# andr345/frtm-vos

Measured on AMD Instinct MI355X. Metric: segmented frames/sec/GPU (480p, ResNet101, full CG iters), higher is better.
Workload: dtype f32

## Files before the change

### frtm-vos_amd/_hip.py

```python
import ctypes
import os

import torch

_HERE = os.path.dirname(os.path.abspath(__file__))
LIB_PATH = os.path.join(_HERE, 'libfrtm_hip.so')

P, I, F, D = ctypes.c_void_p, ctypes.c_int, ctypes.c_float, ctypes.c_double


class ConvDesc(ctypes.Structure):
    _fields_ = [(k, I) for k in ('B', 'Cin', 'Hin', 'Win', 'Cout', 'ksize', 'stride', 'pad',
                                 'relu', 'out_transposed', 'splitk', 'tile', 'w_layout', 'ws_elems', 'w_pitch')]


SIGNATURES = {
    'frtm_last_error': (ctypes.c_char_p, []),
    'frtm_version': (I, []),
    'frtm_device_info': (I, [P]),
    'frtm_pixel_weights': (I, [P, I, I, I, I, F, P, P, P]),
    'frtm_normal_build': (I, [P, I, P, I, I, I, I, I, F, P, I, P, P, P, P, P]),
    'frtm_memory_next_slot': (I, [P, I, F, I, P, P, I, P]),
    'frtm_memory_insert': (I, [P, P, I, P, P]),
    'frtm_filter_scores': (I, [P, P, I, I, I, I, P, I, P]),
# ... 82 lines not shown
    'frtm_bn_stats': (I, [P, I, I, I, F, F, I, P, P, P, P, P, P]),
    'frtm_bn_apply_relu': (I, [P, P, P, P, P, I, I, I, P, P]),
    'frtm_bn_relu_backward': (I, [P, P, P, P, P, P, I, I, I, I, P, P, P, P, P]),
    'frtm_relu_backward': (I, [P, P, ctypes.c_size_t, P, P]),
    'frtm_pyrup2x_backward': (I, [P, I, I, I, P, P, P]),
    'frtm_bilinear_backward': (I, [P, I, I, I, I, I, P, P, P]),
    'frtm_cab_backward_reduce': (I, [P, P, I, I, P, P, P]),
    'frtm_cab_gate_backward': (I, [P, P, P, P, P, P, P, P, I, I, P, P, P, P, P, P, P]),
    'frtm_cab_backward_shallow': (I, [P, P, P, I, I, P, P]),
    'frtm_add_plane': (I, [P, P, F, I, I, P]),
    'frtm_shift9': (I, [P, I, I, I, P, P]),
    'frtm_cab_gate': (I, [P, P, I, P, P, P, P, I, I, P, P]),
    'frtm_project_tail_fits': (I, [I, I, I, I, I]),
    'frtm_project_tail': (I, [P, I, I, I, I, P, P, I, I, P, P]),
    'frtm_tap_mix': (I, [P, I, I, I, P, P, P]),
    'frtm_bicubic_resize': (I, [P, I, I, I, P, I, I, P]),
    'frtm_project_tail_bicubic': (I, [P, I, I, I, I, P, P, I, I, P, P]),
    'frtm_warp_affine': (I, [P, I, I, I, P, I, I, P, I, P]),
    'frtm_warp_affine_u8': (I, [P, I, I, I, P, I, I, P, I, P]),
    'frtm_warp_mask_batch': (I, [P, I, I, P, I, I, P, I, P, P]),
    'frtm_fill32': (I, [P, ctypes.c_size_t, ctypes.c_uint, P]),
    'frtm_label_mask': (I, [P, I, ctypes.c_size_t, P, P, P]),
    'frtm_mask_stats': (I, [P, I, I, I, P, P]),
    'frtm_aug_prepare': (I, [P, P, I, I, P, P, P, P, P]),
    'frtm_pull_push_fill': (I, [P, ctypes.c_size_t, I, I, P]),
    'frtm_pull_push_elems': (ctypes.c_size_t, [I, I]),
    'frtm_aug_transforms': (I, [P, I, P, I, I, P, P, P]),
    'frtm_warp_mask_batch_dev': (I, [P, I, I, P, I, I, P, I, P, P]),
    'frtm_warp_affine_batch': (I, [P, I, I, I, P, I, I, P, P, I, P]),
    'frtm_aug_blend': (I, [P, P, I, I, I, P, P, P, P, P]),
# ... 247 lines not shown
```

### frtm-vos_amd/build.py

```python
import os
import subprocess
import sys

HERE = os.path.dirname(os.path.abspath(__file__))
CSRC = os.path.join(HERE, 'csrc')
LIB = os.path.join(HERE, 'libfrtm_hip.so')
SOURCES = ['target_model.hip', 'target_apply_grouped.hip', 'cg_persistent.hip', 'joint_persistent.hip', 'joint_fit.hip', 'wide_maps.hip', 'conv_igemm.hip', 'conv_gemm32.hip', 'conv_wino.hip', 'conv_wino4.hip', 'conv_bf16x3.hip', 'conv_bf16x1.hip', 'conv3x3_bf16x1.hip', 'conv3x3s2_bf16x1.hip', 'conv_wgrad_bf16x1.hip', 'backbone.hip', 'image_ops.hip', 'refiner_ops.hip', 'refiner_train.hip', 'ragged_group.hip', 'telea_host.hip', 'jf_eval.hip', 'train_step.hip', 'frame_resize.hip', 'native_size.hip']
HIPCC = os.environ.get('HIPCC', '/opt/rocm/bin/hipcc')
FLAGS = ['--offload-arch=gfx950', '-O3', '-std=c++17', '-fPIC', '-Wall', '-Wno-unused-function']
if os.environ.get('FRTM_BUILD_ABLATE'):
    FLAGS.append('-DFRTM_DEBUG_ABLATE')


def _stale(target, deps):
    if not os.path.exists(target):
        return True
    t = os.path.getmtime(target)
    return any(os.path.getmtime(d) > t for d in deps)


def build(force=False, verbose=True):
    headers = [os.path.join(CSRC, 'frtm_common.h'), os.path.join(CSRC, 'conv_common.h'), os.path.join(CSRC, 'resident_grid.h'), os.path.join(CSRC, 'resample_taps.h'), os.path.join(CSRC, 'trunk_route.h'), os.path.join(os.path.dirname(HERE), 'include', 'frtm_hip.h'), __file__]
    objs = []
    for src in SOURCES:
        sp = os.path.join(CSRC, src)
        if not os.path.exists(sp):
            continue
        obj = os.path.join(CSRC, src.replace('.hip', '.o'))
        objs.append(obj)
        if force or _stale(obj, [sp] + headers):
            cmd = [HIPCC] + FLAGS + ['-c', sp, '-o', obj]
            if verbose:
                print(' '.join(cmd), flush=True)
            subprocess.check_call(cmd)
    if force or _stale(LIB, objs):
        cmd = [HIPCC, '--offload-arch=gfx950', '-shared', '-fPIC'] + objs + ['-o', LIB]
        if verbose:
# ... 8 lines not shown
```

### frtm-vos_amd/csrc/refiner_ops.hip

```cpp
#include "frtm_common.h"
#include "resample_taps.h"
#include "../../include/frtm_hip.h"

__global__ __launch_bounds__(256) void k_bilinear_resize(const float* __restrict__ in, int h, int w, float* __restrict__ out, int H, int W,
                                                          int planes, int planes_per_z) {
  const int pix = blockIdx.x * 256 + threadIdx.x;
  if (pix >= H * W) return;
  const int y = pix / W, x = pix - y * W;
  int y0, y1, x0, x1; float ly0, ly1, lx0, lx1;
  bilinear_taps(y, (float)h / (float)H, h, y0, y1, ly0, ly1);
  bilinear_taps(x, (float)w / (float)W, w, x0, x1, lx0, lx1);
  const float w00 = ly0 * lx0, w01 = ly0 * lx1, w10 = ly1 * lx0, w11 = ly1 * lx1;
  const int o00 = y0 * w + x0, o01 = y0 * w + x1, o10 = y1 * w + x0, o11 = y1 * w + x1;
  const int p0 = blockIdx.y * planes_per_z, p1 = min(planes, p0 + planes_per_z);
  const size_t hw = (size_t)h * w, HW = (size_t)H * W;
  for (int pl = p0; pl < p1; ++pl) {
    const float* p = in + pl * hw;
    out[pl * HW + pix] = w00 * p[o00] + w01 * p[o01] + w10 * p[o10] + w11 * p[o11];
  }
}

#define INJ_TH 8
#define INJ_TW 32
#define INJ_CG 4
// ... 143 lines not shown
  const float* p = in + (size_t)blockIdx.x * HW;
  float acc = 0.f;
  if ((HW & 3) == 0 && ((size_t)p & 15) == 0) {
    const float4* p4 = (const float4*)p;
    float a0 = 0.f, a1 = 0.f, a2 = 0.f, a3 = 0.f;
    for (int i = threadIdx.x; i < HW / 4; i += 256) { const float4 v = p4[i]; a0 += v.x; a1 += v.y; a2 += v.z; a3 += v.w; }
    acc = (a0 + a1) + (a2 + a3);
  } else {
    for (int i = threadIdx.x; i < HW; i += 256) acc += p[i];
  }
  acc = block_sum(acc, red);
  if (threadIdx.x == 0) out[blockIdx.x] = acc / (float)HW;
}


#define PT_TH 16
#define PT_TW 64
#define PT_UR 22
#define PT_UC 76
#define PT_YR (PT_UR / 2 + 5)
#define PT_YC (PT_UC / 2 + 5)
#define PT_ZR (PT_TH + 2)
#define PT_ZC (PT_TW + 2)
#define PT_CG 2

__device__ __forceinline__ float pyr_taps(int odd, float a, float b, float c, float d) {
  const float E0 = PYR2X_E0, E1 = PYR2X_E1, E2 = PYR2X_E2, E3 = PYR2X_E3;
  return odd ? E0 * a + E1 * b + E2 * c + E3 * d : E3 * a + E2 * b + E1 * c + E0 * d;
}

__global__ __launch_bounds__(256, 4) void k_project_tail(const float* __restrict__ y, int C, int h, int w, const float* __restrict__ wgt,
                                                       const float* __restrict__ bias, float* __restrict__ out, int Ho, int Wo) {
  constexpr int NY = PT_YR * PT_YC, NYL = (PT_CG * NY + 255) / 256;
  constexpr int NZ = PT_ZR * PT_ZC, NZL = (NZ + 255) / 256;
  __shared__ float ybuf[PT_CG][PT_YR][PT_YC];
  __shared__ float ub[PT_CG][PT_UR][PT_UC];
  __shared__ float zb[PT_CG][PT_ZR][PT_ZC + 1];
  __shared__ int ri0[PT_ZR], ri1[PT_ZR], cj0[PT_ZC], cj1[PT_ZC];
  __shared__ float rl0[PT_ZR], rl1[PT_ZR], cl0[PT_ZC], cl1[PT_ZC];
  __shared__ int org[2];
  const int tid = threadIdx.x, n = blockIdx.z;
  const int Y0 = blockIdx.y * PT_TH, X0 = blockIdx.x * PT_TW;
  const int Hu = 2 * h, Wu = 2 * w;
  if (tid < PT_ZR) {
// ... 413 lines not shown
```

### frtm-vos_amd/csrc/target_model.hip

```cpp
#include "frtm_common.h"
#include "resample_taps.h"
#include "../../include/frtm_hip.h"

__device__ __forceinline__ void hinge_weights(float px, float HW, float tf, float& wf, float& wb) {
  if (tf < 0.f) { wf = 1.f; wb = 1.f; return; }
  float af = px / HW;
  if (px < 10.f) af = tf;
  const float tfe = (af > tf) ? af : tf;
  wf = tfe / af;
  wb = (1.f - tfe) / (1.f - af);
}

template <bool U8>
__device__ __forceinline__ float load_label(const void* p, size_t i) {
  if (U8) return (float)((const unsigned char*)p)[i];
  return ((const float*)p)[i];
}

template <bool U8, bool THRESH>
__global__ __launch_bounds__(256) void k_label_sum(const void* __restrict__ y, int HW, float* __restrict__ partial) {
  __shared__ float red[16];
  const int n = blockIdx.y, part = blockIdx.x;
  const size_t base = (size_t)n * HW;
  const int per = (HW + FRTM_PX_PARTS - 1) / FRTM_PX_PARTS;
// ... 652 lines not shown
__global__ __launch_bounds__(256) void k_transpose2d(const float* __restrict__ in, int rows, int cols, float* __restrict__ out) {
  __shared__ float tile[32][33];
  const int bx = blockIdx.x * 32, by = blockIdx.y * 32;
  const int tx = threadIdx.x & 31, ty = threadIdx.x >> 5;
  for (int k = ty; k < 32; k += 8) {
    const int r = by + k, c = bx + tx;
    tile[k][tx] = (r < rows && c < cols) ? in[(size_t)r * cols + c] : 0.f;
  }
  __syncthreads();
  for (int k = ty; k < 32; k += 8) {
    const int c = bx + k, r = by + tx;
    if (r < rows && c < cols) out[(size_t)c * rows + r] = tile[tx][k];
  }
}

#define MERGE_MAX 16
__global__ __launch_bounds__(256) void k_merge_masks(float* __restrict__ masks, int K, int HW) {
  masks += (size_t)blockIdx.y * K * HW;
  for (int i = blockIdx.x * 256 + threadIdx.x; i < HW; i += gridDim.x * 256) {
    float p[MERGE_MAX];
    float bg = INFINITY;
    for (int k = 1; k < K; ++k) {
      float v = masks[(size_t)k * HW + i];
      v = fminf(fmaxf(v, 1e-7f), 1.f - 1e-7f);
      p[k] = v;
      bg = fminf(bg, 1.f - v);
    }
    p[0] = bg;
    float mx = -INFINITY; int arg = 0;
    for (int k = 0; k < K; ++k) { p[k] = p[k] / (1.f - p[k]); if (p[k] > mx) { mx = p[k]; arg = k; } }
    float den = 0.f;
// ... 46 lines not shown
  if (threadIdx.x == 0) {
    const int tot = (wsum[0] + wsum[1]) + (wsum[2] + wsum[3]);
    if (tot) atomicAdd(&count[k], tot);
  }
}

__global__ __launch_bounds__(256) void k_track_merge(const float* __restrict__ logits, int n, int HW, float* __restrict__ masks,
                                                     unsigned char* __restrict__ labels, const unsigned char* __restrict__ lut, int single,
                                                     int* __restrict__ counts, float thr) {
  const int K = n + 1, f = blockIdx.y;
  logits += (size_t)f * n * HW;
  masks += (size_t)f * K * HW;
  int cnt[MERGE_MAX];
#pragma unroll
  for (int k = 0; k < MERGE_MAX; ++k) cnt[k] = 0;
  for (int i = blockIdx.x * 256 + threadIdx.x; i < HW; i += gridDim.x * 256) {
    float p[MERGE_MAX];
    float bg = INFINITY;
    for (int k = 1; k < K; ++k) {
      const float x = logits[(size_t)(k - 1) * HW + i];
      float v = 1.f / (1.f + expf(-x));
      v = fminf(fmaxf(v, 1e-7f), 1.f - 1e-7f);
      p[k] = v;
      bg = fminf(bg, 1.f - v);
    }
    p[0] = bg;
    float mx = -INFINITY; int arg = 0;
    for (int k = 0; k < K; ++k) { p[k] = p[k] / (1.f - p[k]); if (p[k] > mx) { mx = p[k]; arg = k; } }
    float den = 0.f;
    for (int k = 0; k < K; ++k) { p[k] = expf(p[k] - mx); den += p[k]; }
    const float win = p[arg] / den;
    for (int k = 0; k < K; ++k) masks[(size_t)k * HW + i] = (k == arg) ? win : 0.f;
    if (win > thr) {
#pragma unroll
      for (int k = 0; k < MERGE_MAX; ++k) cnt[k] += (k == arg) ? 1 : 0;
    }
    if (labels) {
      int lab;
      if (single) lab = (arg == 1 && win > 0.5f) ? 1 : 0;
      else {
        const float v = fminf(fmaxf(win, 1e-7f), 1.f - 1e-7f), z = 1e-7f;
        float b2 = INFINITY;
        for (int k = 1; k < K; ++k) b2 = fminf(b2, 1.f - ((k == arg) ? v : z));
        float m2 = -INFINITY; lab = 0;
        for (int k = 0; k < K; ++k) {
          const float q = (k == 0) ? b2 : ((k == arg) ? v : z);
          const float o = q / (1.f - q);
          if (o > m2) { m2 = o; lab = k; }
        }
      }
      labels[(size_t)f * HW + i] = lut[lab];
    }
  }
  if (counts) {
    __shared__ int wsum[4][MERGE_MAX];
    for (int k = 0; k < K; ++k) {
      int c = cnt[k];
#pragma unroll
      for (int off = 32; off > 0; off >>= 1) c += __shfl_xor(c, off, 64);
      if ((threadIdx.x & 63) == 0) wsum[threadIdx.x >> 6][k] = c;
    }
    __syncthreads();
    if (threadIdx.x < K) {
      const int tot = (wsum[0][threadIdx.x] + wsum[1][threadIdx.x]) + (wsum[2][threadIdx.x] + wsum[3][threadIdx.x]);
      if (tot) atomicAdd(&counts[(size_t)f * K + threadIdx.x], tot);
    }
  }
}

static thread_local char g_err[512] = "";
void frtm_set_error(const char* fmt, ...) {
  va_list ap;
  va_start(ap, fmt);
  vsnprintf(g_err, sizeof(g_err), fmt, ap);
  va_end(ap);

}

extern "C" {

const char* frtm_last_error(void) { return g_err; }
int frtm_version(void) { return 100; }
// ... 301 lines not shown
```

### frtm-vos_amd/model/seg_network.py

```python
import torch
from torch import nn
from torch.nn import functional as F

from .. import _hip as H
from .. import ops
from ..lib.utils import conv, relu, interpolate


def _bicubic_phase(d):
    x = (d + torch.arange(-1, 3, dtype=torch.float32)).abs()
    a = -0.75
    near = (a + 2) * x ** 3 - (a + 3) * x ** 2 + 1
    far = a * x ** 3 - 5 * a * x ** 2 + 8 * a * x - 4 * a
    return torch.where(x < 1, near, torch.where(x < 2, far, torch.zeros_like(x)))


_SIDE = {}


def _shared_side_stream(dev):
    key = torch.device(dev).index
    if key not in _SIDE:
        _SIDE[key] = torch.cuda.Stream(device=dev)
    return _SIDE[key]
# ... 119 lines not shown
        self.CAB = nn.ModuleDict()
        self.RRB2 = nn.ModuleDict()
        for L, fc in self.ft_channels.items():
            self.TSE[L] = TSE(fc, in_channels, out_channels)
            self.RRB1[L] = RRB(out_channels, use_bn=use_bn)
            self.CAB[L] = CAB(out_channels, L == 'layer5')
            self.RRB2[L] = RRB(out_channels, use_bn=use_bn)
        self.project = _HEADS[upsampler](out_channels)
        self.use_graphs = False
        self.parallel_eager = True
        self._graphs = {}
        self._pack_key = None
        self.use_winograd = True
        self.fuse_tail = True
        self.mix_taps = True
        self.parallel_levels = True
        self._side = None
        self._pool = None
        self._uses = {}
        self.capture_after = 1

    @property
    def precision(self):
        return self._precision

    @precision.setter
    def precision(self, value):
        if value not in PRECISIONS:
            raise ValueError('precision must be one of %s, not %r' % (PRECISIONS, value))
        self._precision = value
# ... 19 lines not shown
        super().__setattr__(name, value)

    def _apply(self, fn, *a, **k):
        self.invalidate()
        return super()._apply(fn, *a, **k)

    def load_state_dict(self, *a, **k):
        self.invalidate()
        return super().load_state_dict(*a, **k)

    def precompute(self, features):
        red = {L: self.TSE[L].reduce(features[L]) for L in self.ft_channels}
        first = next(iter(self.ft_channels))
        return red, F.adaptive_avg_pool2d(red[first], (1, 1))

    def forward(self, scores, features, image_size, shared=None, frame_of=None):
        if frame_of is not None:
            frames = features[next(iter(self.ft_channels))].shape[0]
            if scores.shape[0] != frame_of.n or frames != frame_of.F:
                raise ValueError('scores (%d samples) and taps (%d frames) do not match the table: %d frames of %r objects'
                                 % (scores.shape[0], frames, frame_of.F, frame_of.counts))
        if scores.is_cuda and shared is None:
            if self.training or torch.is_grad_enabled():
                raise RuntimeError('SegNetwork.forward on the GPU is the inference path (HIP kernels, no autograd): call it in eval() mode '
                                   'under torch.no_grad(); for training / gradients call forward_torch(...) explicitly '
                                   '(the PyTorch definition of the same network) or forward_train(...) (HIP kernels with autograd)')
            if self.use_graphs and frame_of is None:
                return self._forward_graphed(scores, features, image_size)
            par = (self.parallel_levels and self.parallel_eager and next(iter(features.values())).shape[0] >= 2
                   and not torch.cuda.is_current_stream_capturing())
            return self._forward_hip(scores, features, image_size, self._side_streams() if par else None, frame_of)
        return self.forward_torch(scores, features, image_size, shared, frame_of)

    def forward_torch(self, scores, features, image_size, shared=None, frame_of=None):
        red, pool = shared if shared is not None else self.precompute(features)
        group = scores.shape[0] // pool.shape[0]
        if frame_of is not None:
            idx = frame_of.frame_of.to(scores.device)
            red = {L: t.index_select(0, idx) for L, t in red.items()}
            pool = pool.index_select(0, idx)
        elif pool.shape[0] > 1:
            red = {L: t.repeat_interleave(group, 0) for L, t in red.items()}
            pool = pool.repeat_interleave(group, 0)
        x = None
        for i, L in enumerate(self.ft_channels):
            s = interpolate(scores, red[L].shape[-2:])
            h = self.TSE[L](red[L], s)
# ... 112 lines not shown

    def _rrb_hip(self, x, r):
        a = self._conv(x, r['c1'])
        return self._conv(self._conv(a, r['b0']), r['b1'], residual=a)

    def _branch(self, L, p, ft, scores, deepest, table=None):
        group = scores.shape[0] // ft.shape[0]
        h = self._conv(self._conv(ft, p['r0']), p['r2'])
        pool0 = ops.plane_mean(h) if deepest else None
        base = self._conv(h, p['base'])
        t0 = ops.tse_inject(base, p['b0'], p['ws'], scores, group) if table is None else ops.tse_inject_indexed(base, p['b0'], p['ws'], scores, table)
        t = self._conv(self._conv(t0, p['t2']), p['t4'])
        r = self._rrb_hip(t, p['rrb1'])
        return r, ops.plane_mean(r), pool0, (h, base, t0, t)

    def _forward_hip(self, scores, features, image_size, side_streams=None, table=None):
        P = self._packed()
        scores = scores.float().contiguous()
        n = scores.shape[0]
        frames = features[next(iter(self.ft_channels))].shape[0]
        if table is None and n % frames != 0:
            raise ValueError('scores (%d samples) must hold the same number of objects for each of the %d frames' % (n, frames))
        group = n // frames
        levels = list(self.ft_channels)
        cur = torch.cuda.current_stream()
        keep, br = [], {}
        self._capture_events = []

        def order(waiter, waited):
            ev = torch.cuda.Event()
            ev.record(waited)
# ... 11 lines not shown
                    br[L] = self._branch(L, P[L], ft, scores, i == 0, table)
        x, pool0 = None, br[levels[0]][2]
        for i, L in enumerate(levels):
            p = P[L]
            st = side_streams[i] if (side_streams and i < len(side_streams)) else None
            if st is not None:
                order(cur, st)
            r, sp, _, tmp = br[L]
            keep.append(tmp)
            out, gate, dp = cab_level(r, sp, x, pool0, (p['cab_w1'], p['cab_b1'], p['cab_w2'], p['cab_b2']), group, table)
            keep.append((x, gate, out, dp))
            x = self._rrb_hip(out, p['rrb2'])
        pj = P['project']
        u1 = ops.pyrup2x(x)
        y = self._conv(u1, pj['c1'])
        return project_head(y, pj['w2'], pj['b2'], image_size, pj['kind'] == 'bicubic', self.fuse_tail, self.mix_taps and y.shape[1] > 9, pj['eye9'])


def cab_level(r, sp, x, pool0, weights, group, table=None):
    deepest = x is None
    dp = pool0 if deepest else ops.plane_mean(x)
    w1t, b1, w2t, b2 = weights
    if deepest and table is not None:
        gate = ops.cab_gate_indexed(sp, dp, w1t, b1, w2t, b2, table)
        return ops.cab_combine_indexed(r, gate, pool0, table), gate, dp
    gate = ops.cab_gate(sp, dp, w1t, b1, w2t, b2, group if deepest else 0)
    return ops.cab_combine(r, gate, pool0 if deepest else x, group if deepest else 0), gate, dp


def project_head(y, w2, b2, image_size, bicubic, fused, mixed, eye9=None):
    n, _, h, w = y.shape
    size = (int(image_size[-2]), int(image_size[-1]))
    if fused and ops.project_tail_fits(h, w, size, bicubic):
        if mixed:
            ym = ops.tap_mix(y, w2)
            return ops.project_tail(ym, torch.eye(9, device=y.device) if eye9 is None else eye9, b2, size, bicubic)
        return ops.project_tail(y, w2, b2, size, bicubic)
    if bicubic:
        z = ops.bicubic_resize(y, size)
    else:
        u2 = ops.pyrup2x(y)
        z = u2 if size == (2 * h, 2 * w) else ops.bilinear_resize(u2, size)
    out = b2.view(1, 1, 1, 1).expand(n, 1, *size).contiguous()
    return ops.filter_scores(z, w2, out=out, accumulate=True)


def bicubic_tail_fits(h, w, Ho, Wo):
    return ops.project_tail_fits(h, w, (Ho, Wo), bicubic=True)
```

### frtm-vos_amd/ops.py

```python
import ctypes
import functools

import torch

from . import _hip as H

_workspaces = {}


def workspace(device, elems):
    if torch.cuda.is_current_stream_capturing():
        return torch.empty(int(elems), device=device, dtype=torch.float32)
    key = (device, H.stream())
    w = _workspaces.get(key)
    if w is None or w.numel() < elems:
        w = torch.empty(int(elems), device=device, dtype=torch.float32)
        _workspaces[key] = w
    return w


def padded_rows(K):
    return (K + 31) // 32 * 32


# ... 340 lines not shown
def project_tail_fits(h, w, size, bicubic=False):
    return _tail_fits(int(bool(bicubic)), int(h), int(w), int(size[-2]), int(size[-1]))


def project_tail(y, w3x3, bias, size, bicubic=False):
    s = y.shape
    Ho, Wo = int(size[-2]), int(size[-1])
    if not (len(s) == 4 and Ho > 0 and Wo > 0 and w3x3.numel() == 9 * s[1] and y.dtype is w3x3.dtype is _F32
            and (bias is None or (bias.numel() == 1 and bias.dtype is _F32))):
        _refuse('project_tail', 'expected y (n,C,h,w), w3x3 (1,C,3,3), bias (1) or None and a positive size, not %s' % ((Ho, Wo),),
                y=y, w3x3=w3x3, bias=bias)
    n, c, h, w = s
    out = torch.empty(n, 1, Ho, Wo, device=y.device)
    H.call('frtm_project_tail_bicubic' if bicubic else 'frtm_project_tail', H.ptr(y), n, c, h, w, H.ptr(w3x3), H.ptr(bias), Ho, Wo, H.ptr(out))
    return out


def conv_wgrad(dy, x, k, weight=True, bias=True, bf16x1=False):
    B, Cout, Hh, Ww = dy.shape
    Cin = x.shape[1]
    assert tuple(x.shape) == (B, Cin, Hh, Ww) and (weight or bias)
    if bf16x1 and k != 3:
        raise ValueError('conv_wgrad: the bf16x1 form is a 3x3 weight gradient (k = 3), got k = %d' % k)
    elems = H.lib().frtm_conv_wgrad_bf16x1_ws_elems(B, Cout, Cin, Hh, Ww) if bf16x1 else H.lib().frtm_conv_wgrad_ws_elems(B, Cout, Cin, k, Hh, Ww)
    ws = torch.empty(elems, device=dy.device)
    dw = torch.empty(Cout, Cin, k, k, device=dy.device) if weight else None
    db = torch.empty(Cout, device=dy.device) if bias else None
    if bf16x1:
        H.call('frtm_conv_wgrad_bf16x1', H.ptr(dy), H.ptr(x), B, Cout, Cin, Hh, Ww, H.ptr(dw), H.ptr(db), H.ptr(ws), ws.numel())
    else:
# ... 336 lines not shown
```

### include/frtm_hip.h

```cpp
#ifndef FRTM_HIP_H
#define FRTM_HIP_H

#ifdef __cplusplus
extern "C" {
#endif

typedef void* frtm_stream_t;
typedef struct frtm_backbone frtm_backbone_t;

const char* frtm_last_error(void);
int frtm_version(void);
int frtm_device_info(int* out4_host);


#define FRTM_PX_PARTS 32
int frtm_pixel_weights(const void* y, int y_is_u8, int n, int H, int W, float tf,
                       float* out, float* scratch, frtm_stream_t stream);

int frtm_normal_build(const void* labels, int labels_is_u8, const float* pw, int n, int H, int W, int h, int w,
                      float tf, const int* slot_dev, int slot_host, float* Bmem, float* cmem,
                      float* scratch, const int* px_count_dev, frtm_stream_t stream);

int frtm_memory_update_window(float* sw, int cap, float lr, int num_samp_is_zero, int* state, const int* counts, int count_stride,
                              int min_count, int W, int* slots, const float* features, float* samples, int len, const float* labels,
// ... 191 lines not shown
                            int C, int h, int w, int H, int W, float* out, frtm_stream_t stream);
int frtm_cab_gate_indexed(const float* sp, const float* dp, const int* row_of, int rows, const float* W1, const float* b1, const float* W2,
                          const float* b2, int n, int oc, float* gate, frtm_stream_t stream);
int frtm_cab_combine_indexed(const float* shallow, const float* gate, const float* deeper, const int* entry_of, int entries, int n, int C,
                             int hd, int wd, int H, int W, float* out, frtm_stream_t stream);
int frtm_track_merge_ragged(const float* logits, int frames, const int* first, int HW, float* masks, int* counts, float thr,
                            frtm_stream_t stream);
int frtm_pyrup2x(const float* in, int planes, int h, int w, float* out, frtm_stream_t stream);
int frtm_project_tail_fits(int bicubic, int h, int w, int Ho, int Wo);
int frtm_project_tail(const float* y, int n, int C, int h, int w, const float* w3x3, const float* bias, int Ho, int Wo, float* out,
                      frtm_stream_t stream);
int frtm_tap_mix(const float* y, int n, int C, int hw, const float* w3x3, float* out, frtm_stream_t stream);
int frtm_bicubic_resize(const float* in, int planes, int h, int w, float* out, int H, int W, frtm_stream_t stream);
int frtm_project_tail_bicubic(const float* y, int n, int C, int h, int w, const float* w3x3, const float* bias, int Ho, int Wo, float* out,
                              frtm_stream_t stream);
int frtm_plane_mean(const float* in, int planes, int HW, float* out, frtm_stream_t stream);

size_t frtm_conv_wgrad_ws_elems(int B, int Cout, int Cin, int k, int H, int W);
int frtm_conv_wgrad(const float* dy, const float* x, int B, int Cout, int Cin, int k, int H, int W, float* dw, float* dbias, float* ws,
                    size_t ws_elems, frtm_stream_t stream);
size_t frtm_conv_wgrad_bf16x1_ws_elems(int B, int Cout, int Cin, int H, int W);
int frtm_conv_wgrad_bf16x1(const float* dy, const float* x, int B, int Cout, int Cin, int H, int W, float* dw, float* dbias, float* ws,
                           size_t ws_elems, frtm_stream_t stream);
long frtm_conv_wgrad_bf16x1_launches(void);
int frtm_bn_stats(const float* x, int N, int C, int HW, float eps, float factor, int train, float* rmean, float* rvar, float* mean,
                  float* invstd, double* part, frtm_stream_t stream);
int frtm_bn_apply_relu(const float* x, const float* mean, const float* invstd, const float* gamma, const float* beta, int N, int C, int HW,
                       float* out, frtm_stream_t stream);
int frtm_bn_relu_backward(const float* dy, const float* out, const float* x, const float* mean, const float* invstd, const float* gamma,
                          int N, int C, int HW, int train, float* dx, float* dgamma, float* dbeta, double* part, frtm_stream_t stream);
// ... 72 lines not shown
```

Baseline: 662.0.

## Add tap-specialised projection tail kernel and optional fused tail+mask-merge kernel

Adds a specialised kernel for the refiner's final projection after tap mixing. It reads the 9 pre-mixed tap planes directly and sums shifted bilinear-upsampled planes, with no 3x3 weight multiply, processing three taps per pass. An optional merge variant also fuses the per-frame object mask merge, labelling and counts into the same kernel. The taps path is on by default and the merge path is off, so the extra complexity and the changed rounding order bring some numerical and maintenance risk.

```diff
diff --git a/frtm-vos_amd/_hip.py b/frtm-vos_amd/_hip.py
--- a/frtm-vos_amd/_hip.py
+++ b/frtm-vos_amd/_hip.py
@@ -120,6 +120,9 @@
     'frtm_project_tail_fits': (I, [I, I, I, I, I]),
     'frtm_project_tail': (I, [P, I, I, I, I, P, P, I, I, P, P]),
     'frtm_tap_mix': (I, [P, I, I, I, P, P, P]),
+    'frtm_project_tail_taps': (I, [P, I, I, I, P, I, I, P, P]),
+    'frtm_project_tail_merge_max_objects': (I, []),
+    'frtm_project_tail_merge': (I, [P, I, I, I, I, P, I, I, P, P, P, I, P, F, P]),
     'frtm_bicubic_resize': (I, [P, I, I, I, P, I, I, P]),
     'frtm_project_tail_bicubic': (I, [P, I, I, I, I, P, P, I, I, P, P]),
     'frtm_warp_affine': (I, [P, I, I, I, P, I, I, P, I, P]),
diff --git a/frtm-vos_amd/build.py b/frtm-vos_amd/build.py
--- a/frtm-vos_amd/build.py
+++ b/frtm-vos_amd/build.py
@@ -5,7 +5,7 @@
 HERE = os.path.dirname(os.path.abspath(__file__))
 CSRC = os.path.join(HERE, 'csrc')
 LIB = os.path.join(HERE, 'libfrtm_hip.so')
-SOURCES = ['target_model.hip', 'target_apply_grouped.hip', 'cg_persistent.hip', 'joint_persistent.hip', 'joint_fit.hip', 'wide_maps.hip', 'conv_igemm.hip', 'conv_gemm32.hip', 'conv_wino.hip', 'conv_wino4.hip', 'conv_bf16x3.hip', 'conv_bf16x1.hip', 'conv3x3_bf16x1.hip', 'conv3x3s2_bf16x1.hip', 'conv_wgrad_bf16x1.hip', 'backbone.hip', 'image_ops.hip', 'refiner_ops.hip', 'refiner_train.hip', 'ragged_group.hip', 'telea_host.hip', 'jf_eval.hip', 'train_step.hip', 'frame_resize.hip', 'native_size.hip']
+SOURCES = ['target_model.hip', 'target_apply_grouped.hip', 'cg_persistent.hip', 'joint_persistent.hip', 'joint_fit.hip', 'wide_maps.hip', 'conv_igemm.hip', 'conv_gemm32.hip', 'conv_wino.hip', 'conv_wino4.hip', 'conv_bf16x3.hip', 'conv_bf16x1.hip', 'conv3x3_bf16x1.hip', 'conv3x3s2_bf16x1.hip', 'conv_wgrad_bf16x1.hip', 'backbone.hip', 'image_ops.hip', 'refiner_ops.hip', 'refiner_head.hip', 'refiner_train.hip', 'ragged_group.hip', 'telea_host.hip', 'jf_eval.hip', 'train_step.hip', 'frame_resize.hip', 'native_size.hip']
 HIPCC = os.environ.get('HIPCC', '/opt/rocm/bin/hipcc')
 FLAGS = ['--offload-arch=gfx950', '-O3', '-std=c++17', '-fPIC', '-Wall', '-Wno-unused-function']
 if os.environ.get('FRTM_BUILD_ABLATE'):
@@ -20,7 +20,7 @@
 
 
 def build(force=False, verbose=True):
-    headers = [os.path.join(CSRC, 'frtm_common.h'), os.path.join(CSRC, 'conv_common.h'), os.path.join(CSRC, 'resident_grid.h'), os.path.join(CSRC, 'resample_taps.h'), os.path.join(CSRC, 'trunk_route.h'), os.path.join(os.path.dirname(HERE), 'include', 'frtm_hip.h'), __file__]
+    headers = [os.path.join(CSRC, 'frtm_common.h'), os.path.join(CSRC, 'conv_common.h'), os.path.join(CSRC, 'resident_grid.h'), os.path.join(CSRC, 'resample_taps.h'), os.path.join(CSRC, 'refiner_tail.h'), os.path.join(CSRC, 'track_merge.h'), os.path.join(CSRC, 'trunk_route.h'), os.path.join(os.path.dirname(HERE), 'include', 'frtm_hip.h'), __file__]
     objs = []
     for src in SOURCES:
         sp = os.path.join(CSRC, src)
diff --git a/frtm-vos_amd/csrc/refiner_head.hip b/frtm-vos_amd/csrc/refiner_head.hip
--- /dev/null
+++ b/frtm-vos_amd/csrc/refiner_head.hip
@@ -0,0 +1,222 @@
+#include "frtm_common.h"
+#include "refiner_tail.h"
+#include "track_merge.h"
+#include "../../include/frtm_hip.h"
+
+#define TT_CG 3
+#define TT_ZP (PT_ZC + 1)
+#define TT_LG (4 * 256)
+
+__device__ __forceinline__ float taps_chain(bool second_first, float c0, float a, float c1, float b, float c2, float c, float c3, float d) {
+#pragma clang fp contract(off)
+  float s = second_first ? __builtin_fmaf(c1, b, c0 * a) : __builtin_fmaf(c0, a, c1 * b);
+  s = __builtin_fmaf(c2, c, s);
+  return __builtin_fmaf(c3, d, s);
+}
+__device__ __forceinline__ float bilinear_sum(float w00, float u00, float w01, float u01, float w10, float u10, float w11, float u11) {
+#pragma clang fp contract(off)
+  return ((w00 * u00 + w01 * u01) + w10 * u10) + w11 * u11;
+}
+
+constexpr unsigned long long TT_VFORM = 0xffff0ffffa5ull;
+static_assert(2 * PT_UR <= 64, "one bit per u row and parity");
+__device__ __forceinline__ float taps_chain(bool second_first, int odd, float a, float b, float c, float d) {
+  const float E0 = PYR2X_E0, E1 = PYR2X_E1, E2 = PYR2X_E2, E3 = PYR2X_E3;
+  return odd ? taps_chain(second_first, E0, a, E1, b, E2, c, E3, d) : taps_chain(second_first, E3, a, E2, b, E1, c, E0, d);
+}
+
+template <bool MERGE>
+__device__ __forceinline__ void tail_taps_tile(const float* __restrict__ y, int s0, int n_obj, int h, int w, const float* __restrict__ bias,
+                                               float* __restrict__ out, int Ho, int Wo, float* __restrict__ lgt, int frame,
+                                               float* __restrict__ masks, unsigned char* __restrict__ labels, const unsigned char* __restrict__ lut,
+                                               int single, int* __restrict__ counts, float thr) {
+  constexpr int NY = PT_YR * PT_YC, NYL = (TT_CG * NY + 255) / 256;
+  constexpr int NZ = PT_ZR * PT_ZC, NZL = (NZ + 255) / 256;
+  static_assert(TT_CG * NY <= TT_CG * PT_ZR * TT_ZP, "the y patch is staged in the z buffer");
+  __shared__ float ub[TT_CG][PT_UR][PT_UC];
+  __shared__ float zy[TT_CG * PT_ZR * TT_ZP];
+  __shared__ int ri0[PT_ZR], ri1[PT_ZR], cj0[PT_ZC], cj1[PT_ZC];
+  __shared__ float rl0[PT_ZR], rl1[PT_ZR], cl0[PT_ZC], cl1[PT_ZC];
+  const int tid = threadIdx.x;
+  const int Y0 = blockIdx.y * PT_TH, X0 = blockIdx.x * PT_TW;
+  const int Hu = 2 * h, Wu = 2 * w;
+  if (tid < PT_ZR) {
+    const int zy_ = Y0 - 1 + tid;
+    int i0 = -1, i1 = -1; float l0 = 0.f, l1 = 0.f;
+    if (zy_ >= 0 && zy_ < Ho) bilinear_taps(zy_, (float)Hu / (float)Ho, Hu, i0, i1, l0, l1);
+    ri0[tid] = i0; ri1[tid] = i1; rl0[tid] = l0; rl1[tid] = l1;
+  }
+  if (tid >= 64 && tid < 64 + PT_ZC) {
+    const int j = tid - 64, zx = X0 - 1 + j;
+    int i0 = -1, i1 = -1; float l0 = 0.f, l1 = 0.f;
+    if (zx >= 0 && zx < Wo) bilinear_taps(zx, (float)Wu / (float)Wo, Wu, i0, i1, l0, l1);
+    cj0[j] = i0; cj1[j] = i1; cl0[j] = l0; cl1[j] = l1;
+  }
+  int ur0, uc0;
+  { int i1; float l0, l1;
+    bilinear_taps(max(Y0 - 1, 0), (float)Hu / (float)Ho, Hu, ur0, i1, l0, l1);
+    bilinear_taps(max(X0 - 1, 0), (float)Wu / (float)Wo, Wu, uc0, i1, l0, l1); }
+  __syncthreads();
+  const int yr0 = (ur0 >> 1) - 2, yc0 = (uc0 >> 1) - 2;
+  int a_goff[NYL];
+#pragma unroll
+  for (int k = 0; k < NYL; ++k) {
+    const int e = tid + k * 256;
+    const int g = e / NY, r = (e - g * NY) / PT_YC, cc = e - g * NY - r * PT_YC;
+    a_goff[k] = e < TT_CG * NY ? g * (h * w) + min(max(yr0 + r, 0), h - 1) * w + min(max(yc0 + cc, 0), w - 1) : -1;
+  }
+  const int bc_g = tid / PT_UC, bc_j = tid - bc_g * PT_UC;
+  const bool bc_on = tid < TT_CG * PT_UC;
+  const int bc_odd = (uc0 + bc_j) & 1, bc_b = ((uc0 + bc_j) >> 1) - 2 + bc_odd - yc0;
+  const int par = ur0 & 1;
+  static_assert(PT_UR * PT_UC < (1 << 11) && PT_ZR * TT_ZP < (1 << 11), "packed stage D offsets");
+  int d_pk[NZL];
+  float d_w00[NZL], d_w01[NZL], d_w10[NZL], d_w11[NZL];
+#pragma unroll
+  for (int k = 0; k < NZL; ++k) {
+    const int e = tid + k * 256;
+    const int i = e / PT_ZC, j = e - i * PT_ZC;
+    const bool ok = e < NZ && ri0[e < NZ ? i : 0] >= 0 && cj0[j] >= 0;
+    const int ii = e < NZ ? i : 0;
+    const int a0 = ok ? ri0[ii] - ur0 : 0, a1 = ok ? ri1[ii] - ur0 : 0, b0 = ok ? cj0[j] - uc0 : 0, b1 = ok ? cj1[j] - uc0 : 0;
+    d_pk[k] = e < NZ ? ((i * TT_ZP + j) << 13) | ((a1 - a0) << 12) | ((b1 - b0) << 11) | (a0 * PT_UC + b0) : -1;
+    d_w00[k] = ok ? rl0[ii] * cl0[j] : 0.f; d_w01[k] = ok ? rl0[ii] * cl1[j] : 0.f;
+    d_w10[k] = ok ? rl1[ii] * cl0[j] : 0.f; d_w11[k] = ok ? rl1[ii] * cl1[j] : 0.f;
+  }
+  const int tx = tid & 63, ty = tid >> 6;
+  const size_t hw = (size_t)h * w;
+  const float b = bias ? bias[0] : 0.f;
+  float pre[NYL];
+  auto fetch = [&](int obj, int trip) {
+    const float* yp = y + ((size_t)(s0 + obj) * 9 + (size_t)trip * TT_CG) * hw;
+#pragma unroll
+    for (int k = 0; k < NYL; ++k) pre[k] = a_goff[k] >= 0 ? yp[a_goff[k]] : 0.f;
+  };
+  fetch(0, 0);
+  for (int obj = 0; obj < n_obj; ++obj) {
+    float acc[4] = {0.f, 0.f, 0.f, 0.f};
+    for (int trip = 0; trip < 3; ++trip) {
+      const bool last = obj + 1 == n_obj && trip == 2;
+#pragma unroll
+      for (int k = 0; k < NYL; ++k) if (a_goff[k] >= 0) zy[tid + k * 256] = pre[k];
+      __syncthreads();
+      if (!last) fetch(trip == 2 ? obj + 1 : obj, trip == 2 ? 0 : trip + 1);
+      if (bc_on) {
+        float hxv[PT_YR];
+#pragma unroll
+        for (int r = 0; r < PT_YR; ++r) {
+          const float* v = &zy[bc_g * NY + r * PT_YC + bc_b];
+          hxv[r] = taps_chain(true, bc_odd, v[0], v[1], v[2], v[3]);
+        }
+        if (par == 0) {
+#pragma unroll
+          for (int i = 0; i < PT_UR; ++i) {
+            const int odd = i & 1, bb = (i >> 1) + odd;
+            ub[bc_g][i][bc_j] = taps_chain((TT_VFORM >> i) & 1, odd, hxv[bb], hxv[bb + 1], hxv[bb + 2], hxv[bb + 3]);
+          }
+        } else {
+#pragma unroll
+          for (int i = 0; i < PT_UR; ++i) {
+            const int odd = (i + 1) & 1, bb = ((i + 1) >> 1) + odd;
+            ub[bc_g][i][bc_j] = taps_chain((TT_VFORM >> (PT_UR + i)) & 1, odd, hxv[bb], hxv[bb + 1], hxv[bb + 2], hxv[bb + 3]);
+          }
+        }
+      }
+      __syncthreads();
+#pragma unroll
+      for (int g = 0; g < TT_CG; ++g) {
+        const float* up = &ub[g][0][0];
+#pragma unroll
+        for (int k = 0; k < NZL; ++k)
+          if (d_pk[k] >= 0) {
+            int pk = d_pk[k];
+            asm volatile("" : "+v"(pk));
+            const int o00 = pk & 0x7ff, o01 = o00 + ((pk >> 11) & 1), o10 = o00 + ((pk >> 12) & 1) * PT_UC, o11 = o10 + o01 - o00;
+            zy[g * PT_ZR * TT_ZP + (pk >> 13)] = bilinear_sum(d_w00[k], up[o00], d_w01[k], up[o01], d_w10[k], up[o10], d_w11[k], up[o11]);
+          }
+      }
+      __syncthreads();
+#pragma unroll
+      for (int g = 0; g < TT_CG; ++g)
+#pragma unroll
+        for (int o = 0; o < 4; ++o) acc[o] = acc[o] + zy[(g * PT_ZR + ty * 4 + o + trip) * TT_ZP + tx + g];
+      if (!last) __syncthreads();
+    }
+#pragma unroll
+    for (int o = 0; o < 4; ++o) {
+      const int yy = Y0 + ty * 4 + o, xx = X0 + tx;
+      if (MERGE) lgt[(obj * 4 + o) * 256 + tid] = acc[o] + b;
+      else if (yy < Ho && xx < Wo) out[((size_t)s0 * Ho + yy) * Wo + xx] = acc[o] + b;
+    }
+  }
+  if (MERGE) {
+    const int K = n_obj + 1;
+    const size_t HW = (size_t)Ho * Wo;
+    int cnt[MERGE_MAX];
+#pragma unroll
+    for (int k = 0; k < MERGE_MAX; ++k) cnt[k] = 0;
+    for (int o = 0; o < 4; ++o) {
+      const int yy = Y0 + ty * 4 + o, xx = X0 + tx;
+      if (yy < Ho && xx < Wo) {
+        const size_t i = (size_t)yy * Wo + xx;
+        track_merge_pixel([&](int k) { return lgt[((k - 1) * 4 + o) * 256 + tid]; }, K, masks + (size_t)frame * K * HW + i, HW,
+                          labels ? labels + (size_t)frame * HW + i : nullptr, lut, single, thr, cnt);
+      }
+    }
+    if (counts) track_merge_counts(cnt, K, counts + (size_t)frame * K);
+  }
+}
+
+__global__ __launch_bounds__(256, 4) void k_project_tail_taps(const float* __restrict__ y, int h, int w, const float* __restrict__ bias,
+                                                            float* __restrict__ out, int Ho, int Wo) {
+  tail_taps_tile<false>(y, blockIdx.z, 1, h, w, bias, out, Ho, Wo, nullptr, 0, nullptr, nullptr, nullptr, 0, nullptr, 0.f);
+}
+
+__global__ __launch_bounds__(256, 2) void k_project_tail_merge(const float* __restrict__ y, int n_obj, int h, int w, const float* __restrict__ bias,
+                                                             int Ho, int Wo, float* __restrict__ masks, unsigned char* __restrict__ labels,
+                                                             const unsigned char* __restrict__ lut, int single, int* __restrict__ counts, float thr) {
+  extern __shared__ float lgt[];
+  tail_taps_tile<true>(y, blockIdx.z * n_obj, n_obj, h, w, bias, nullptr, Ho, Wo, lgt, blockIdx.z, masks, labels, lut, single, counts, thr);
+}
+
+extern "C" {
+
+int frtm_project_tail_taps(const float* ym, int n, int h, int w, const float* bias, int Ho, int Wo, float* out, frtm_stream_t stream) {
+  FRTM_CHECK_ARG(ym && out && n > 0 && h > 1 && w > 1 && Ho > 0 && Wo > 0, "frtm_project_tail_taps: bad argument");
+  FRTM_CHECK_ARG(n <= 65535, "frtm_project_tail_taps: at most 65535 samples per call (got %d)", n);
+  FRTM_CHECK_ARG((size_t)9 * h * w < 0x7fffffff, "frtm_project_tail_taps: map too large");
+  FRTM_CHECK_ARG(frtm_project_tail_fits(0, h, w, Ho, Wo),
+                 "frtm_project_tail_taps: resize ratio %.3f x %.3f outside the fused kernel's patch (use pyrup2x + bilinear_resize + filter_scores)",
+                 2.0 * h / Ho, 2.0 * w / Wo);
+  FRTM_CHECK_ARG(ceil_div(Ho, PT_TH) <= 65535, "frtm_project_tail_taps: at most %d output rows (got %d)", 65535 * PT_TH, Ho);
+  dim3 g(ceil_div(Wo, PT_TW), ceil_div(Ho, PT_TH), n);
+  k_project_tail_taps<<<g, 256, 0, (hipStream_t)stream>>>(ym, h, w, bias, out, Ho, Wo);
+  FRTM_LAUNCH_CHECK();
+  return FRTM_OK;
+}
+
+int frtm_project_tail_merge_max_objects(void) { return FRTM_TAIL_MERGE_MAX_OBJECTS; }
+
+int frtm_project_tail_merge(const float* ym, int frames, int n_obj, int h, int w, const float* bias, int Ho, int Wo, float* masks,
+                            unsigned char* labels, const unsigned char* lut, int single_object_decode, int* counts, float thr,
+                            frtm_stream_t stream) {
+  FRTM_CHECK_ARG(ym && masks && frames > 0 && h > 1 && w > 1 && Ho > 0 && Wo > 0 && (labels == nullptr || lut != nullptr),
+                 "frtm_project_tail_merge: bad argument");
+  FRTM_CHECK_ARG(n_obj >= 1 && n_obj <= FRTM_TAIL_MERGE_MAX_OBJECTS,
+                 "frtm_project_tail_merge: 1 to %d objects per frame (got %d; more: frtm_project_tail_taps + frtm_track_merge)",
+                 FRTM_TAIL_MERGE_MAX_OBJECTS, n_obj);
+  FRTM_CHECK_ARG(frames <= 65535, "frtm_project_tail_merge: at most 65535 frames per call (got %d)", frames);
+  FRTM_CHECK_ARG((size_t)9 * h * w < 0x7fffffff, "frtm_project_tail_merge: map too large");
+  FRTM_CHECK_ARG(frtm_project_tail_fits(0, h, w, Ho, Wo),
+                 "frtm_project_tail_merge: resize ratio %.3f x %.3f outside the fused kernel's patch", 2.0 * h / Ho, 2.0 * w / Wo);
+  FRTM_CHECK_ARG(ceil_div(Ho, PT_TH) <= 65535, "frtm_project_tail_merge: at most %d output rows (got %d)", 65535 * PT_TH, Ho);
+  hipStream_t st = (hipStream_t)stream;
+  if (counts) FRTM_HIP(hipMemsetAsync(counts, 0, sizeof(int) * (size_t)frames * (n_obj + 1), st));
+  dim3 g(ceil_div(Wo, PT_TW), ceil_div(Ho, PT_TH), frames);
+  k_project_tail_merge<<<g, 256, (size_t)n_obj * TT_LG * sizeof(float), st>>>(ym, n_obj, h, w, bias, Ho, Wo, masks, labels, lut,
+                                                                            single_object_decode, counts, thr);
+  FRTM_LAUNCH_CHECK();
+  return FRTM_OK;
+}
+
+}
diff --git a/frtm-vos_amd/csrc/refiner_ops.hip b/frtm-vos_amd/csrc/refiner_ops.hip
--- a/frtm-vos_amd/csrc/refiner_ops.hip
+++ b/frtm-vos_amd/csrc/refiner_ops.hip
@@ -1,5 +1,6 @@
 #include "frtm_common.h"
 #include "resample_taps.h"
+#include "refiner_tail.h"
 #include "../../include/frtm_hip.h"
 
 __global__ __launch_bounds__(256) void k_bilinear_resize(const float* __restrict__ in, int h, int w, float* __restrict__ out, int H, int W,
@@ -181,20 +182,7 @@
 }
 
 
-#define PT_TH 16
-#define PT_TW 64
-#define PT_UR 22
-#define PT_UC 76
-#define PT_YR (PT_UR / 2 + 5)
-#define PT_YC (PT_UC / 2 + 5)
-#define PT_ZR (PT_TH + 2)
-#define PT_ZC (PT_TW + 2)
 #define PT_CG 2
-
-__device__ __forceinline__ float pyr_taps(int odd, float a, float b, float c, float d) {
-  const float E0 = PYR2X_E0, E1 = PYR2X_E1, E2 = PYR2X_E2, E3 = PYR2X_E3;
-  return odd ? E0 * a + E1 * b + E2 * c + E3 * d : E3 * a + E2 * b + E1 * c + E0 * d;
-}
 
 __global__ __launch_bounds__(256, 4) void k_project_tail(const float* __restrict__ y, int C, int h, int w, const float* __restrict__ wgt,
                                                        const float* __restrict__ bias, float* __restrict__ out, int Ho, int Wo) {
diff --git a/frtm-vos_amd/csrc/refiner_tail.h b/frtm-vos_amd/csrc/refiner_tail.h
--- /dev/null
+++ b/frtm-vos_amd/csrc/refiner_tail.h
@@ -0,0 +1,16 @@
+#pragma once
+#include "resample_taps.h"
+
+#define PT_TH 16
+#define PT_TW 64
+#define PT_UR 22
+#define PT_UC 76
+#define PT_YR (PT_UR / 2 + 5)
+#define PT_YC (PT_UC / 2 + 5)
+#define PT_ZR (PT_TH + 2)
+#define PT_ZC (PT_TW + 2)
+
+__device__ __forceinline__ float pyr_taps(int odd, float a, float b, float c, float d) {
+  const float E0 = PYR2X_E0, E1 = PYR2X_E1, E2 = PYR2X_E2, E3 = PYR2X_E3;
+  return odd ? E0 * a + E1 * b + E2 * c + E3 * d : E3 * a + E2 * b + E1 * c + E0 * d;
+}
diff --git a/frtm-vos_amd/csrc/target_model.hip b/frtm-vos_amd/csrc/target_model.hip
--- a/frtm-vos_amd/csrc/target_model.hip
+++ b/frtm-vos_amd/csrc/target_model.hip
@@ -1,5 +1,6 @@
 #include "frtm_common.h"
 #include "resample_taps.h"
+#include "track_merge.h"
 #include "../../include/frtm_hip.h"
 
 __device__ __forceinline__ void hinge_weights(float px, float HW, float tf, float& wf, float& wb) {
@@ -690,7 +691,6 @@
   }
 }
 
-#define MERGE_MAX 16
 __global__ __launch_bounds__(256) void k_merge_masks(float* __restrict__ masks, int K, int HW) {
   masks += (size_t)blockIdx.y * K * HW;
   for (int i = blockIdx.x * 256 + threadIdx.x; i < HW; i += gridDim.x * 256) {
@@ -767,58 +767,10 @@
   int cnt[MERGE_MAX];
 #pragma unroll
   for (int k = 0; k < MERGE_MAX; ++k) cnt[k] = 0;
-  for (int i = blockIdx.x * 256 + threadIdx.x; i < HW; i += gridDim.x * 256) {
-    float p[MERGE_MAX];
-    float bg = INFINITY;
-    for (int k = 1; k < K; ++k) {
-      const float x = logits[(size_t)(k - 1) * HW + i];
-      float v = 1.f / (1.f + expf(-x));
-      v = fminf(fmaxf(v, 1e-7f), 1.f - 1e-7f);
-      p[k] = v;
-      bg = fminf(bg, 1.f - v);
-    }
-    p[0] = bg;
-    float mx = -INFINITY; int arg = 0;
-    for (int k = 0; k < K; ++k) { p[k] = p[k] / (1.f - p[k]); if (p[k] > mx) { mx = p[k]; arg = k; } }
-    float den = 0.f;
-    for (int k = 0; k < K; ++k) { p[k] = expf(p[k] - mx); den += p[k]; }
-    const float win = p[arg] / den;
-    for (int k = 0; k < K; ++k) masks[(size_t)k * HW + i] = (k == arg) ? win : 0.f;
-    if (win > thr) {
-#pragma unroll
-      for (int k = 0; k < MERGE_MAX; ++k) cnt[k] += (k == arg) ? 1 : 0;
-    }
-    if (labels) {
-      int lab;
-      if (single) lab = (arg == 1 && win > 0.5f) ? 1 : 0;
-      else {
-        const float v = fminf(fmaxf(win, 1e-7f), 1.f - 1e-7f), z = 1e-7f;
-        float b2 = INFINITY;
-        for (int k = 1; k < K; ++k) b2 = fminf(b2, 1.f - ((k == arg) ? v : z));
-        float m2 = -INFINITY; lab = 0;
-        for (int k = 0; k < K; ++k) {
-          const float q = (k == 0) ? b2 : ((k == arg) ? v : z);
-          const float o = q / (1.f - q);
-          if (o > m2) { m2 = o; lab = k; }
-        }
-      }
-      labels[(size_t)f * HW + i] = lut[lab];
-    }
-  }
-  if (counts) {
-    __shared__ int wsum[4][MERGE_MAX];
-    for (int k = 0; k < K; ++k) {
-      int c = cnt[k];
-#pragma unroll
-      for (int off = 32; off > 0; off >>= 1) c += __shfl_xor(c, off, 64);
-      if ((threadIdx.x & 63) == 0) wsum[threadIdx.x >> 6][k] = c;
-    }
-    __syncthreads();
-    if (threadIdx.x < K) {
-      const int tot = (wsum[0][threadIdx.x] + wsum[1][threadIdx.x]) + (wsum[2][threadIdx.x] + wsum[3][threadIdx.x]);
-      if (tot) atomicAdd(&counts[(size_t)f * K + threadIdx.x], tot);
-    }
-  }
+  for (int i = blockIdx.x * 256 + threadIdx.x; i < HW; i += gridDim.x * 256)
+    track_merge_pixel([&](int k) { return logits[(size_t)(k - 1) * HW + i]; }, K, masks + i, (size_t)HW, labels ? labels + (size_t)f * HW + i : nullptr,
+                      lut, single, thr, cnt);
+  if (counts) track_merge_counts(cnt, K, counts + (size_t)f * K);
 }
 
 static thread_local char g_err[512] = "";
diff --git a/frtm-vos_amd/csrc/track_merge.h b/frtm-vos_amd/csrc/track_merge.h
--- /dev/null
+++ b/frtm-vos_amd/csrc/track_merge.h
@@ -0,0 +1,60 @@
+#pragma once
+#include "frtm_common.h"
+
+#define MERGE_MAX 16
+
+template <class Logit>
+__device__ __forceinline__ void track_merge_pixel(Logit logit, int K, float* __restrict__ masks, size_t HW, unsigned char* __restrict__ label,
+                                                  const unsigned char* __restrict__ lut, int single, float thr, int (&cnt)[MERGE_MAX]) {
+  float p[MERGE_MAX];
+  float bg = INFINITY;
+  for (int k = 1; k < K; ++k) {
+    const float x = logit(k);
+    float v = 1.f / (1.f + expf(-x));
+    v = fminf(fmaxf(v, 1e-7f), 1.f - 1e-7f);
+    p[k] = v;
+    bg = fminf(bg, 1.f - v);
+  }
+  p[0] = bg;
+  float mx = -INFINITY; int arg = 0;
+  for (int k = 0; k < K; ++k) { p[k] = p[k] / (1.f - p[k]); if (p[k] > mx) { mx = p[k]; arg = k; } }
+  float den = 0.f;
+  for (int k = 0; k < K; ++k) { p[k] = expf(p[k] - mx); den += p[k]; }
+  const float win = p[arg] / den;
+  for (int k = 0; k < K; ++k) masks[(size_t)k * HW] = (k == arg) ? win : 0.f;
+  if (win > thr) {
+#pragma unroll
+    for (int k = 0; k < MERGE_MAX; ++k) cnt[k] += (k == arg) ? 1 : 0;
+  }
+  if (label) {
+    int lab;
+    if (single) lab = (arg == 1 && win > 0.5f) ? 1 : 0;
+    else {
+      const float v = fminf(fmaxf(win, 1e-7f), 1.f - 1e-7f), z = 1e-7f;
+      float b2 = INFINITY;
+      for (int k = 1; k < K; ++k) b2 = fminf(b2, 1.f - ((k == arg) ? v : z));
+      float m2 = -INFINITY; lab = 0;
+      for (int k = 0; k < K; ++k) {
+        const float q = (k == 0) ? b2 : ((k == arg) ? v : z);
+        const float o = q / (1.f - q);
+        if (o > m2) { m2 = o; lab = k; }
+      }
+    }
+    *label = lut[lab];
+  }
+}
+
+__device__ __forceinline__ void track_merge_counts(const int (&cnt)[MERGE_MAX], int K, int* __restrict__ counts) {
+  __shared__ int wsum[4][MERGE_MAX];
+  for (int k = 0; k < K; ++k) {
+    int c = cnt[k];
+#pragma unroll
+    for (int off = 32; off > 0; off >>= 1) c += __shfl_xor(c, off, 64);
+    if ((threadIdx.x & 63) == 0) wsum[threadIdx.x >> 6][k] = c;
+  }
+  __syncthreads();
+  if (threadIdx.x < K) {
+    const int tot = (wsum[0][threadIdx.x] + wsum[1][threadIdx.x]) + (wsum[2][threadIdx.x] + wsum[3][threadIdx.x]);
+    if (tot) atomicAdd(&counts[threadIdx.x], tot);
+  }
+}
diff --git a/frtm-vos_amd/model/seg_network.py b/frtm-vos_amd/model/seg_network.py
--- a/frtm-vos_amd/model/seg_network.py
+++ b/frtm-vos_amd/model/seg_network.py
@@ -157,6 +157,8 @@
         self.use_winograd = True
         self.fuse_tail = True
         self.mix_taps = True
+        self.merge_tail = False
+        self.tail_taps = True
         self.parallel_levels = True
         self._side = None
         self._pool = None
@@ -206,7 +208,7 @@
         first = next(iter(self.ft_channels))
         return red, F.adaptive_avg_pool2d(red[first], (1, 1))
 
-    def forward(self, scores, features, image_size, shared=None, frame_of=None):
+    def forward(self, scores, features, image_size, shared=None, frame_of=None, merge=None):
         if frame_of is not None:
             frames = features[next(iter(self.ft_channels))].shape[0]
             if scores.shape[0] != frame_of.n or frames != frame_of.F:
@@ -221,8 +223,18 @@
                 return self._forward_graphed(scores, features, image_size)
             par = (self.parallel_levels and self.parallel_eager and next(iter(features.values())).shape[0] >= 2
                    and not torch.cuda.is_current_stream_capturing())
-            return self._forward_hip(scores, features, image_size, self._side_streams() if par else None, frame_of)
+            if merge is not None and (frame_of is not None or not self.takes_merge(scores, features, image_size, merge[1])):
+                merge = None
+            return self._forward_hip(scores, features, image_size, self._side_streams() if par else None, frame_of, merge)
         return self.forward_torch(scores, features, image_size, shared, frame_of)
+
+    def takes_merge(self, scores, features, image_size, n_obj):
+        if not (scores.is_cuda and self.merge_tail and self.tail_taps and self.mix_taps and self.fuse_tail and not self.use_graphs
+                and isinstance(self.project, BackwardCompatibleUpsampler) and self.project.conv2.weight.shape[1] > 9
+                and 1 <= n_obj <= ops.tail_merge_max_objects()):
+            return False
+        h, w = features[list(self.ft_channels)[-1]].shape[-2:]
+        return ops.project_tail_fits(2 * h, 2 * w, image_size)
 
     def forward_torch(self, scores, features, image_size, shared=None, frame_of=None):
         red, pool = shared if shared is not None else self.precompute(features)
@@ -365,7 +377,7 @@
         r = self._rrb_hip(t, p['rrb1'])
         return r, ops.plane_mean(r), pool0, (h, base, t0, t)
 
-    def _forward_hip(self, scores, features, image_size, side_streams=None, table=None):
+    def _forward_hip(self, scores, features, image_size, side_streams=None, table=None, merge=None):
         P = self._packed()
         scores = scores.float().contiguous()
         n = scores.shape[0]
@@ -407,7 +419,8 @@
         pj = P['project']
         u1 = ops.pyrup2x(x)
         y = self._conv(u1, pj['c1'])
-        return project_head(y, pj['w2'], pj['b2'], image_size, pj['kind'] == 'bicubic', self.fuse_tail, self.mix_taps and y.shape[1] > 9, pj['eye9'])
+        return project_head(y, pj['w2'], pj['b2'], image_size, pj['kind'] == 'bicubic', self.fuse_tail, self.mix_taps and y.shape[1] > 9, pj['eye9'],
+                            self.tail_taps, merge)
 
 
 def cab_level(r, sp, x, pool0, weights, group, table=None):
@@ -421,14 +434,21 @@
     return ops.cab_combine(r, gate, pool0 if deepest else x, group if deepest else 0), gate, dp
 
 
-def project_head(y, w2, b2, image_size, bicubic, fused, mixed, eye9=None):
+def project_head(y, w2, b2, image_size, bicubic, fused, mixed, eye9=None, taps=False, merge=None):
     n, _, h, w = y.shape
     size = (int(image_size[-2]), int(image_size[-1]))
     if fused and ops.project_tail_fits(h, w, size, bicubic):
         if mixed:
             ym = ops.tap_mix(y, w2)
+            if taps and not bicubic:
+                if merge is not None:
+                    ops.project_tail_merge(ym, b2, *merge)
+                    return None
+                return ops.project_tail_taps(ym, b2, size)
             return ops.project_tail(ym, torch.eye(9, device=y.device) if eye9 is None else eye9, b2, size, bicubic)
         return ops.project_tail(y, w2, b2, size, bicubic)
+    if merge is not None:
+        raise RuntimeError('project_head: merge handed to a head that does not end in ops.project_tail_merge')
     if bicubic:
         z = ops.bicubic_resize(y, size)
     else:
diff --git a/frtm-vos_amd/ops.py b/frtm-vos_amd/ops.py
--- a/frtm-vos_amd/ops.py
+++ b/frtm-vos_amd/ops.py
@@ -378,6 +378,41 @@
     out = torch.empty(n, 1, Ho, Wo, device=y.device)
     H.call('frtm_project_tail_bicubic' if bicubic else 'frtm_project_tail', H.ptr(y), n, c, h, w, H.ptr(w3x3), H.ptr(bias), Ho, Wo, H.ptr(out))
     return out
+
+
+def project_tail_taps(ym, bias, size):
+    s = ym.shape
+    Ho, Wo = int(size[-2]), int(size[-1])
+    if not (len(s) == 4 and s[1] == 9 and Ho > 0 and Wo > 0 and ym.dtype is _F32 and (bias is None or (bias.numel() == 1 and bias.dtype is _F32))):
+        _refuse('project_tail_taps', 'expected ym (n,9,h,w), bias (1) or None and a positive size, not %s' % ((Ho, Wo),), ym=ym, bias=bias)
+    n, _, h, w = s
+    out = torch.empty(n, 1, Ho, Wo, device=ym.device)
+    H.call('frtm_project_tail_taps', H.ptr(ym), n, h, w, H.ptr(bias), Ho, Wo, H.ptr(out))
+    return out
+
+
+@functools.lru_cache(maxsize=None)
+def tail_merge_max_objects():
+    return int(H.lib().frtm_project_tail_merge_max_objects())
+
+
+def project_tail_merge(ym, bias, frames, n_obj, masks, labels=None, lut=None, single_object=False, counts=None, thr=0.5):
+    s = ym.shape
+    if not (len(s) == 4 and s[1] == 9 and s[0] == frames * n_obj and 1 <= n_obj <= tail_merge_max_objects() and ym.dtype is _F32
+            and masks.dim() >= 2 and masks.dtype is _F32 and (bias is None or (bias.numel() == 1 and bias.dtype is _F32))):
+        _refuse('project_tail_merge', 'expected ym (frames * n_obj,9,h,w) for %d frames of %d objects (at most %d), bias (1) or None and float32 masks'
+                % (frames, n_obj, tail_merge_max_objects()), ym=ym, bias=bias, masks=masks)
+    Hh, Ww = masks.shape[-2:]
+    if not (masks.is_contiguous() and masks.numel() == frames * (n_obj + 1) * Hh * Ww
+            and (labels is None or (labels.is_contiguous() and labels.dtype == torch.uint8 and labels.numel() == frames * Hh * Ww
+                                    and lut is not None and lut.dtype == torch.uint8 and lut.numel() >= n_obj + 1))
+            and (counts is None or (counts.is_contiguous() and counts.dtype == torch.int32 and counts.numel() == frames * (n_obj + 1)))):
+        _refuse('project_tail_merge', 'expected dense masks (frames, n_obj + 1, H, W), uint8 labels (frames, 1, H, W) with a uint8 lut of n_obj + 1 '
+                'entries, int32 counts (frames, n_obj + 1)', masks=masks, labels=labels, lut=lut, counts=counts)
+    H.call('frtm_project_tail_merge', H.ptr(ym), frames, n_obj, s[2], s[3], H.ptr(bias), Hh, Ww, H.ptr(masks),
+           None if labels is None else labels.data_ptr(), None if lut is None else lut.data_ptr(), int(bool(single_object)),
+           None if counts is None else counts.data_ptr(), float(thr))
+    return masks
 
 
 def conv_wgrad(dy, x, k, weight=True, bias=True, bf16x1=False):
diff --git a/include/frtm_hip.h b/include/frtm_hip.h
--- a/include/frtm_hip.h
+++ b/include/frtm_hip.h
@@ -229,6 +229,12 @@
 int frtm_bicubic_resize(const float* in, int planes, int h, int w, float* out, int H, int W, frtm_stream_t stream);
 int frtm_project_tail_bicubic(const float* y, int n, int C, int h, int w, const float* w3x3, const float* bias, int Ho, int Wo, float* out,
                               frtm_stream_t stream);
+int frtm_project_tail_taps(const float* ym, int n, int h, int w, const float* bias, int Ho, int Wo, float* out, frtm_stream_t stream);
+#define FRTM_TAIL_MERGE_MAX_OBJECTS 6
+int frtm_project_tail_merge_max_objects(void);
+int frtm_project_tail_merge(const float* ym, int frames, int n_obj, int h, int w, const float* bias, int Ho, int Wo, float* masks,
+                            unsigned char* labels, const unsigned char* lut, int single_object_decode, int* counts, float thr,
+                            frtm_stream_t stream);
 int frtm_plane_mean(const float* in, int planes, int HW, float* out, frtm_stream_t stream);
 
 size_t frtm_conv_wgrad_ws_elems(int B, int Cout, int Cin, int k, int H, int W);
```

Result: no change. 663.6, median of 3 (+0.2%).
